# IGNF/MAESTRO

Measured on AMD Instinct MI355X. Metric: MAE-pretrain tiles/sec, higher is better.
Workload: dtype bf16

## Files before the change

maestro_amd/csrc/mask.hip:

```cpp
#include "common.hpp"
#include "../../include/maestro_hip.h"

namespace {

__global__ __launch_bounds__(1024) void mask_select_kernel(const float* __restrict__ noise, const uint8_t* __restrict__ smask,
                                                          int* __restrict__ visible_idx, int* __restrict__ masked_idx,
                                                          int* __restrict__ inv, uint8_t* __restrict__ mask, int L, int k) {
    extern __shared__ __attribute__((aligned(16))) float sm[];
    const int L4 = (L + 3) & ~3;
    int* wtot = reinterpret_cast<int*>(sm + L4);
    const int b = blockIdx.x, lane = threadIdx.x & 63, w = threadIdx.x >> 6;
    for (int i = threadIdx.x; i < L4; i += 1024) {
        float v = INFINITY;
        if (i < L) {
            v = noise[(size_t)b * L + i];
            if (smask && smask[(size_t)b * L + i]) v = 0.f;
        }
        sm[i] = v;
    }
    __syncthreads();
    int base = 0;
    for (int i0 = 0; i0 < L; i0 += 1024) {
        const int i = i0 + threadIdx.x;
        int f = 0;
// ... 32 lines not shown
                inv[(size_t)b * L + i] = i - nm;
            }
        }
    }
}

__global__ __launch_bounds__(256) void gather_rows_kernel(const float* __restrict__ src, const int* __restrict__ idx,
                                                          float* __restrict__ dst, int B, int src_L, int n_idx, int dim,
                                                          int dst_L, int dst_off) {
    const int row = blockIdx.x * 4 + (threadIdx.x >> 6), lane = threadIdx.x & 63;
    if (row >= B * n_idx) return;
    const int b = row / n_idx, j = row - b * n_idx;
    const float* s = src + ((size_t)b * src_L + idx[row]) * dim;
    float* d = dst + ((size_t)b * dst_L + dst_off + j) * dim;
    for (int c = lane * 4; c < dim; c += 256) *reinterpret_cast<f32x4*>(d + c) = *reinterpret_cast<const f32x4*>(s + c);
}

constexpr int GC_ROWS = 8;
template <int NV>
__global__ __launch_bounds__(256) void gather_rows_bf16_cs_kernel(const float* __restrict__ src, const int* __restrict__ idx,
                                                                  bf16_t* __restrict__ dst, float* __restrict__ cs_partial, int B,
                                                                  int src_L, int n_idx, int dim) {
    __shared__ f32x4 red[4][64 * NV];
    const int w = threadIdx.x >> 6, lane = threadIdx.x & 63;
    const long rows = (long)B * n_idx, row0 = ((long)blockIdx.x * 4 + w) * GC_ROWS;
    f32x4 v[GC_ROWS][NV], cs[NV];
#pragma unroll
    for (int j = 0; j < NV; ++j) cs[j] = (f32x4){0, 0, 0, 0};
#pragma unroll
    for (int r = 0; r < GC_ROWS; ++r) {
// ... 60 lines not shown
    const int row = blockIdx.x * 4 + (threadIdx.x >> 6), lane = threadIdx.x & 63;
    if (row >= B * L) return;
    const int b = row / L, t = row - b * L;
    const int iv = inv[row];
    const float* s = iv < 0 ? mask_token + (size_t)tok_slot[(size_t)b * slot_stride + t] * Dd : y + ((size_t)b * n_vis + iv) * Dd;
    const float* pr = pos + (size_t)t * Dd;
    const float* dr = date ? date + ((size_t)b * n_date_rows + date_row[t]) * 8 : nullptr;
    float* o = xdec + (size_t)row * Dd;
    for (int c = lane * 4; c < Dd; c += 256) {
        f32x4 v = *reinterpret_cast<const f32x4*>(s + c) + *reinterpret_cast<const f32x4*>(pr + c);
        if (dr && c >= Dd - 8) v += *reinterpret_cast<const f32x4*>(dr + (c - (Dd - 8)));
        *reinterpret_cast<f32x4*>(o + c) = v;
    }
}

constexpr int UM_ROWS = 512, UM_NT = 1024;
template <bool DET>
__global__ __launch_bounds__(UM_NT) void unmask_bwd_token_kernel(const float* __restrict__ dxdec, const uint8_t* __restrict__ mask,
                                                                 const int* __restrict__ tok_slot, float* __restrict__ dmask_token,
                                                                 int B, int L, int Dd, int slot, int t_lo, int t_hi, int slot_stride) {
    __shared__ __attribute__((aligned(16))) float red[UM_NT * 4];
    __shared__ int row_off[UM_ROWS];
    const int span = t_hi - t_lo, total = B * span;
    const int cols = Dd >> 2, lanes = UM_NT / cols;
    const int col = threadIdx.x % cols, sub = threadIdx.x / cols;
    const int r0 = blockIdx.x * UM_ROWS;
    for (int rr = threadIdx.x; rr < UM_ROWS; rr += UM_NT) {
        const int r = r0 + rr;
        int off = -1;
        if (r < total) {
// ... 108 lines not shown
    MH_LAUNCH_CHECK();
    return 0;
}

extern "C" int mh_unmask_assemble_per_sample(const float* y, const int* inv, const float* mask_token, const int* tok_slot_bl,
                                             const float* pos, const float* date, const int* date_row, int n_date_rows,
                                             float* xdec, int B, int L, int n_vis, int Dd, void* stream) {
    MH_CHECK_ARG(y && inv && mask_token && tok_slot_bl && pos && xdec && Dd % 4 == 0 && Dd >= 8, "mh_unmask_assemble_per_sample: bad arguments");
    MH_CHECK_ARG(!date || date_row, "mh_unmask_assemble_per_sample: date without date_row");
    hipLaunchKernelGGL(unmask_kernel, dim3(ceil_div((long)B * L, 4)), dim3(256), 0, (hipStream_t)stream, y, inv, mask_token,
                       tok_slot_bl, pos, date, date_row, n_date_rows, xdec, B, L, n_vis, Dd, L);
    MH_LAUNCH_CHECK();
    return 0;
}

extern "C" int mh_unmask_token_grad(const float* dxdec, const uint8_t* mask, const int* tok_slot, float* dmask_token, int B,
                                    int L, int Dd, int slot, int t_lo, int t_hi, void* stream) {
    MH_CHECK_ARG(dxdec && mask && tok_slot && dmask_token && Dd % 4 == 0 && Dd <= 1024, "mh_unmask_token_grad: bad arguments");
    MH_CHECK_ARG(0 <= t_lo && t_lo < t_hi && t_hi <= L, "mh_unmask_token_grad: bad token range");
    hipLaunchKernelGGL(unmask_bwd_token_kernel<false>, dim3(ceil_div((long)B * (t_hi - t_lo), UM_ROWS)), dim3(UM_NT), 0,
                       (hipStream_t)stream, dxdec, mask, tok_slot, dmask_token, B, L, Dd, slot, t_lo, t_hi, 0);
    MH_LAUNCH_CHECK();
    return 0;
}

extern "C" int mh_unmask_token_grad_per_sample(const float* dxdec, const uint8_t* mask, const int* tok_slot_bl, float* dmask_token,
                                               int B, int L, int Dd, int slot, void* stream) {
    MH_CHECK_ARG(dxdec && mask && tok_slot_bl && dmask_token && Dd % 4 == 0 && Dd <= 1024 && B > 0 && L > 0,
                 "mh_unmask_token_grad_per_sample: bad arguments");
    hipLaunchKernelGGL(unmask_bwd_token_kernel<false>, dim3(ceil_div((long)B * L, UM_ROWS)), dim3(UM_NT), 0, (hipStream_t)stream, dxdec, mask,
// ... 44 lines not shown
```

maestro_amd/csrc/norm.hip:

```cpp
#include "gemm_common.hpp"
#include <type_traits>

namespace {

struct RowMap { int L, off; };
__device__ __forceinline__ size_t map_row(RowMap m, int b, int j) { return (size_t)b * m.L + m.off + j; }

template <int NV>
__global__ __launch_bounds__(256) void ln_fwd_kernel(const float* __restrict__ x, RowMap xm, const float* __restrict__ gamma,
                                                     const float* __restrict__ beta, void* __restrict__ y, RowMap ym,
                                                     int y_is_f32, float* __restrict__ mean, float* __restrict__ rstd,
                                                     int B, int n, int dim, float eps, uint8_t* __restrict__ y8,
                                                     const float* __restrict__ y8_scale, float* __restrict__ y8_amax,
                                                     uint8_t* __restrict__ y8s, int ld_y8s) {
    const int row = blockIdx.x * 4 + (threadIdx.x >> 6);
    const int lane = threadIdx.x & 63;
    if (row >= B * n) return;
    const int b = row / n, j = row - b * n;
    const float* xr = x + map_row(xm, b, j) * dim;
    const int nv = dim >> 2;
    f32x4 v[NV];
    float s = 0.f;
#pragma unroll
    for (int i = 0; i < NV; ++i) {
// ... 121 lines not shown
            *reinterpret_cast<uint32_t*>(y8 + yrow + 4 * (lane + 64 * i)) = pack_e4m3x4(q, mx_inv_scale(sbyte));
            if ((lane & 7) == 0) y8s[map_row(ym, b, j) * ld_y8s + ((lane + 64 * i) >> 3)] = (uint8_t)sbyte;
        }
        if constexpr (FP8) {
#pragma unroll
            for (int e = 0; e < 4; ++e) amax8 = amax_fold(amax8, o[e]);
            *reinterpret_cast<uint32_t*>(y8 + yrow + 4 * (lane + 64 * i)) = pack_e4m3x4(o, s8);
        }
    }
    if (lane == 0) { mean[row] = mu; rstd[row] = rs; }
    if constexpr (FP8) {
        if (y8_amax) {
            amax8 = wave_amax(amax8);
            if (lane == 0 && amax_nonzero(amax8)) atomic_max_pos(y8_amax, amax8);
        }
    }
}

constexpr int ROWS_PER_WAVE = 4;

template <int NV, bool FULL>
__device__ __forceinline__ void ln_bwd_store_partial(float* red, float* __restrict__ partial, const f32x4 (&gsum)[NV],
                                                     const f32x4 (&bsum)[NV], const f32x4 (&csum)[NV], int w, int lane, int dim) {
    float* rg = red + (size_t)w * 3 * dim;
#pragma unroll
    for (int i = 0; i < NV; ++i) {
        const int c = lane + 64 * i;
        if (FULL || c < (dim >> 2)) {
            *reinterpret_cast<f32x4*>(rg + 4 * c) = gsum[i];
            *reinterpret_cast<f32x4*>(rg + dim + 4 * c) = bsum[i];
// ... 281 lines not shown
    MH_CHECK_ARG(!y8s || (dim % 32 == 0 && !y_is_f32), "mh_layernorm_fwd_mx: dim %% 32 == 0 required, got %d", dim);
    if (nvs <= 4 && dim == 256 * nvs && !y_is_f32) {
        auto fast = [&](auto y8_form) {
            ln_for_nv<false>(nvs, [&](auto nv) {
                hipLaunchKernelGGL((ln_fwd_fast_kernel<decltype(nv)::value, decltype(y8_form)::value>), grid, block, 0, s, x, xm, gamma,
                                   beta, (bf16_t*)y, ym, mean, rstd, B, n, eps, (uint8_t*)y8, y8_scale, y8_amax, (uint8_t*)y8s, ld_y8s);
            });
        };
        if (y8s) fast(ln_c<LN_Y8_MX>{}); else if (y8) fast(ln_c<LN_Y8_TENSOR>{}); else fast(ln_c<LN_Y8_NONE>{});
    } else {
        ln_for_nv<true>(nvs, [&](auto nv) {
            hipLaunchKernelGGL(ln_fwd_kernel<decltype(nv)::value>, grid, block, 0, s, x, xm, gamma, beta, y, ym, y_is_f32, mean, rstd, B, n,
                               dim, eps, (uint8_t*)y8, y8_scale, y8_amax, (uint8_t*)y8s, ld_y8s);
        });
    }
    MH_LAUNCH_CHECK();
    return 0;
}

extern "C" long mh_layernorm_bwd_workspace(int rows, int dim) {
    return (long)ceil_div(rows, 4 * ROWS_PER_WAVE) * 3 * dim;
}

static int layernorm_bwd_impl(const void* dy, int dy_L, int dy_off, int dy_is_f32, const float* x, int x_L, int x_off,
                              const float* gamma, const float* mean, const float* rstd, const float* dres, float* dx,
                              void* dx_bf16, float* dgamma, float* dbeta, float* dcol, float* workspace, bool partial_only,
                              int B, int n, int dim, void* stream) {
    const int rows = B * n, nblk = ceil_div(rows, 4 * ROWS_PER_WAVE);
    const size_t lds = (size_t)4 * 3 * dim * sizeof(float);
    dim3 grid(nblk), block(256);
// ... 61 lines not shown
```

maestro_amd/engine.py:

```python

from __future__ import annotations

import contextlib
import gc
import os
import weakref
import time

import torch
from torch import nn

from maestro_amd import hip
from maestro_amd.fp8 import mx_scale_cols, resolve_scaling
from maestro_amd.layers.utils import check_device_mask_config, draw_struct_masks, mask_draw_jobs

F32, BF16, I32, U8 = torch.float32, torch.bfloat16, torch.int32, torch.uint8
_NEVER = object()
_ROCTX = os.environ.get("MAESTRO_ROCTX", "0") == "1"
RING = 4
ALIGN = 64


class ParamStore:

# ... 133 lines not shown
    @property
    def x0(self):
        return self.xs[0]

    @property
    def x_last(self):
        return self.xs[-1]

    @property
    def top16(self):
        return self.saved[-1]["gy16"] if self.depth else self.dx0_16

    def top_bias_grad(self):
        return self.eng.store.g(self.t.layers[-1][1].net[4].bias) if self.depth else None

    def forward(self, before_layer=None) -> None:
        eng, ps, M = self.eng, self.eng.store, self.M
        dim, mlp, inner = self.dim, self.mlp, self.inner
        for l, (attn, ff) in enumerate(self.t.layers):
            if before_layer is not None:
                before_layer(l)
            s, x_in, x_mid, x_out = self.saved[l], self.xs[2 * l], self.xs[2 * l + 1], self.xs[2 * l + 2]
            if self.f8 is not None:
                self._forward_layer_fp8(l, attn, ff, s, x_in, x_mid, x_out)
                continue
            proj = attn.to_out[0]
            hip.layernorm_fwd(x_in, M, 0, attn.norm.weight, attn.norm.bias, s["h1"], M, 0, s["mean1"], s["rstd1"], 1, M, dim)
            hip.gemm(hip.GEMM_NT, M, 3 * inner, dim, s["h1"], dim, ps.h(attn.to_qkv.weight), dim, s["qkv"], 3 * inner)
            hip.attn_fwd(s["qkv"], s["o"], s["lse"], self.Bn, self.N, self.H, self.Dh, attn.scale)
            hip.gemm(hip.GEMM_NT, M, dim, inner, s["o"], inner, ps.h(proj.weight), inner, x_mid, dim,
                     hip.OUT_F32 | hip.BIAS | hip.RESIDUAL, bias=proj.bias, res=x_in, ldr=dim)
            ln2, fc1, fc2 = ff.net[0], ff.net[1], ff.net[4]
            hip.layernorm_fwd(x_mid, M, 0, ln2.weight, ln2.bias, s["h2"], M, 0, s["mean2"], s["rstd2"], 1, M, dim)
            hip.gemm(hip.GEMM_NT, M, mlp, dim, s["h2"], dim, ps.h(fc1.weight), dim, s["act"], mlp,
                     hip.BIAS | hip.GELU | hip.AUX_DGELU | eng.aux_flag, bias=fc1.bias, aux_out=s["hpre"], ldaux=mlp)
            hip.gemm(hip.GEMM_NT, M, dim, mlp, s["act"], mlp, ps.h(fc2.weight), mlp, x_out, dim,
                     hip.OUT_F32 | hip.BIAS | hip.RESIDUAL, bias=fc2.bias, res=x_mid, ldr=dim)

    def _forward_layer_fp8(self, l, attn, ff, s, x_in, x_mid, x_out) -> None:
        eng, M, dim, mlp, inner = self.eng, self.M, self.dim, self.mlp, self.inner
        plan, f = eng.fp8, self.f8[l]
        proj, ln2, fc1, fc2 = attn.to_out[0], ff.net[0], ff.net[1], ff.net[4]
# ... 243 lines not shown

def resolve_deterministic(flag: bool | None = None) -> bool:
    if flag is None:
        return os.environ.get("MAESTRO_DETERMINISTIC", "0") == "1"
    return bool(flag)


def resolve_mask_rng(mode: str | None = None) -> str:
    if mode is None:
        mode = os.environ.get("MAESTRO_MASK_RNG") or "host"
    if mode not in ("host", "device"):
        raise ValueError(f"mask_rng={mode!r}: expected 'host' or 'device'")
    return mode


def training_warm_passes() -> int:
    return 0 if _PROCESS_WARMED else max(0, int(os.environ.get("MAESTRO_WARM_PASSES", "6")))


def _retire_graphs(graphs: dict) -> None:
    if graphs:
        _RETIRED_GRAPHS.append(dict(graphs))
        graphs.clear()


def drain_retired_graphs() -> None:
    if _RETIRED_GRAPHS:
        torch.cuda.synchronize()
        _RETIRED_GRAPHS.clear()

# ... 355 lines not shown
        for name in m.enc_to_dec:
            ordered += [(f"enc_to_dec.{name}.{k}", p) for k, p in m.enc_to_dec[name].named_parameters()]
        ordered += [(f"mask_token.{k}", p) for k, p in m.mask_token.items()]
        for name in m.decoder:
            ordered += [(f"decoder.{name}.{k}", p) for k, p in m.decoder[name].named_parameters()]
        for name in m.embed_to_rec:
            ordered += [(f"embed_to_rec.{name}.{k}", p) for k, p in m.embed_to_rec[name].named_parameters()]
        self.store = ParamStore(ordered, device)
        for bname in ("enc_pos_encoding", "dec_pos_encoding"):
            setattr(m, bname, getattr(m, bname).to(device))
        if dtype == "fp8":
            from maestro_amd.fp8 import Fp8Plan
            self.fp8 = Fp8Plan(device, self.store.total, scaling=self.fp8_scaling)
        self._alloc()
        self._alloc_mask_upload()
        if self.fp8 is not None:
            self.fp8.finalize()
        self.store.refresh_half(force=True)
        self._pack_conv_weights()

    @property
    def grad_hook(self):
        return self._grad_hook

    @grad_hook.setter
    def grad_hook(self, fn) -> None:
        if fn is not None and getattr(self, "deterministic", False):
            raise ValueError("deterministic=True excludes a gradient hook / exchange: the order of the cross-rank sum is the "
                             "collective library's, and the ready spans would have to move behind the ordered reduce")
        self._grad_hook = fn
# ... 58 lines not shown
        for g in self.groups:
            Bn, L, N = g.Beff, g.L, g.N
            n_dates = sum(s.D for s in g.mods)
            tok_slot = torch.cat([torch.full((s.n_tok,), s.slot, dtype=I32) for s in g.mods])
            date_row = torch.cat([(s.date_off + torch.arange(s.n_tok) // s.L).to(I32) for s in g.mods])
            pos_dec = torch.cat([m.pos_dec_rows[s.name].repeat(s.D, 1) for s in g.mods], dim=0)
            self.gb[g.name] = dict(
                xg=e(Bn, L, E),
                vis=e(Bn, N, dt=I32), msk=e(Bn, g.k, dt=I32), inv=e(Bn, L, dt=I32), mask=e(Bn, L, dt=U8),
                dates=z(Bn, n_dates, 8), n_dates=n_dates, tok_slot=tok_slot.to(dev), date_row=date_row.to(dev),
                pos_dec=pos_dec.to(dev).contiguous(), tok_table=e(len(g.mods), Dd),
                henc=e(Bn * N, E, dt=BF16), mean_e=e(Bn * N), rstd_e=e(Bn * N), y_e2d=e(Bn * N, Dd),
                dy_e2d=e(Bn * N, Dd), dy_e2d16=e(Bn * N, Dd, dt=BF16), dhenc=e(Bn * N, E, dt=BF16),
                e2d_cs=e(hip.gather_rows_cs_rows(Bn * N), Dd) if self.ends_capable and Dd <= 1024 else None,
                mean_j=e(Bn * N), rstd_j=e(Bn * N))
            holder = m.encoder[g.model]
            self.enc[g.name] = Stack(self, holder, Bn, N, f"enc.{g.name}")
            self.dec[g.name] = Stack(self, m.decoder[g.model], Bn, L, f"dec.{g.name}")
        if m.encoder_inter is not None:
            self.joint = Stack(self, m.encoder_inter, self.B, m.joint_N, "joint")
        else:
            self.joint = None
        for g in self.groups:
            self.gb[g.name]["ln_ws"] = e(max(hip.layernorm_bwd_workspace(g.Beff * g.L, Dd),
                                             hip.layernorm_bwd_workspace(g.Beff * g.N, E)))
        self.loss_acc = z(1)
        srcs = {s.src: s for s in self.mods.values()}
        tot_w = sum(s.Dates * s.L for s in srcs.values())
        self.loss_w = {n: (s.Dates * s.L) / tot_w for n, s in srcs.items()}

    def _alloc_mask_upload(self) -> None:
        segs, off = [], 0
        for g in self.groups:
            for key, dt, esz in (("noise", F32, 4), ("struct", U8, 1)):
                n = g.Beff * g.L * esz
                segs.append((g.name, key, dt, off, n, (g.Beff, g.L)))
                off += (n + 255) // 256 * 256
        self._mask_dev = torch.zeros(off, dtype=U8, device=self.device)
        self._mask_segs = segs
        for name, key, dt, o, n, shape in segs:
            self.gb[name][key] = self._mask_dev[o: o + n].view(dt).view(shape)
        self._mask_stage = self._mask_host = self._upload_stream = self._mask_draw = None
        if self.mask_rng == "device":
            self._mask_draw = hip.MaskDraw(mask_draw_jobs(self.groups, self.mods, self.B),
# ... 237 lines not shown
                part = torch.empty(hip.masked_loss_partial_size(s.Beff, s.n_tok), dtype=F32, device=self.device)
                return part, [(part, self.loss_acc, part.numel(), 1, 1)]
            form, acc = "_det", self.sites.get("fwd", ("loss", s.name), make)
        elif self._loss_cs and b.get("drec_cs") is not None:
            form, cs = "_cs", (b["drec_cs"],)
        bands = () if s.G == 1 else (s.C_src, s.c0, s.C)
        getattr(hip, f"masked_loss{'_bands' if bands else ''}{form}")(
            b["rec"], b["target"], gbuf["mask"], b["cnt"], self.loss_w[s.src], acc, b["drec"], *cs, s.Beff, s.n_tok, g.L, s.tok_off,
            s.K, self.p_loss, *bands)

    def _forward_launches(self, batch: dict) -> None:
        m, E, Dd = self.model, self.E, self.Dd
        self.loss_acc.zero_()
        if self._opt is not None:
            self._opt_launch_stages()

        def head(g):
            def run():
                gbuf, st = self.gb[g.name], self.enc[g.name]
                self._opt_wait("embed")
                for s in g.mods:
                    self.embed[s.name].forward(batch, gbuf, gbuf["xg"], g.L, self.mb[s.name]["target"], self.normalise)
                hip.mask_select(gbuf["noise"], gbuf["struct"], gbuf["vis"], gbuf["msk"], gbuf["inv"], gbuf["mask"], g.Beff,
                                g.L, g.k)
                hip.gather_rows(gbuf["xg"], gbuf["vis"], st.x0, g.Beff, g.L, g.N, E, g.N, 0)
                st.forward(lambda l: self._opt_wait("enc", l))
                head_post(g, gbuf, st)
            return run

        def head_post(g, gbuf, st):
            nrm = st.t.norm
            self._opt_wait("enc", max(st.depth - 1, 0))
            if self.joint is not None:
                hip.layernorm_fwd(st.x_last, g.N, 0, nrm.weight, nrm.bias, self.joint.x0, m.joint_N, g.joint_off,
                                  gbuf["mean_e"], gbuf["rstd_e"], g.Beff, g.N, E)
            else:
                hip.layernorm_fwd(st.x_last, g.N, 0, nrm.weight, nrm.bias, gbuf["y_e2d" if self.e2d_identity else "henc"], g.N, 0,
                                  gbuf["mean_e"], gbuf["rstd_e"], g.Beff, g.N, E)

        def tail(g):
            def run():
                gbuf, st = self.gb[g.name], self.dec[g.name]
                self._opt_wait("e2d")
                if self.joint is not None:
                    nrm = self.joint.t.norm
                    hip.layernorm_fwd(self.joint.x_last, m.joint_N, g.joint_off, nrm.weight, nrm.bias,
                                      gbuf["y_e2d" if self.e2d_identity else "henc"], g.N, 0, gbuf["mean_j"], gbuf["rstd_j"],
                                      g.Beff, g.N, E)
                lin = m.enc_to_dec[g.model]
                M = g.Beff * g.N
                if not self.e2d_identity:
                    hip.gemm(hip.GEMM_NT, M, Dd, E, gbuf["henc"], E, self.store.h(lin.weight), E, gbuf["y_e2d"], Dd,
                             hip.OUT_F32 | hip.BIAS, bias=lin.bias)
                for s in g.mods:
                    gbuf["tok_table"][s.slot].copy_(m.mask_token[s.src].view(s.G, Dd)[s.gi])
                if self.tie_order == "torch":
                    hip.unmask_assemble_per_sample(gbuf["y_e2d"], gbuf["inv"], gbuf["tok_table"], gbuf["tok_slot_ps"], gbuf["pos_dec"],
                                                   gbuf["dates"], gbuf["date_row"], gbuf["n_dates"], st.x0, g.Beff, g.L, g.N, Dd)
                else:
                    hip.unmask_assemble(gbuf["y_e2d"], gbuf["inv"], gbuf["tok_table"], gbuf["tok_slot"], gbuf["pos_dec"],
                                        gbuf["dates"], gbuf["date_row"], gbuf["n_dates"], st.x0, g.Beff, g.L, g.N, Dd)
                st.forward(lambda l: self._opt_wait("dec", l))
                tail_post(g, gbuf, st)
            return run

        def tail_post(g, gbuf, st):
            nrm = st.t.norm
            self._opt_wait("rec")
            for s in g.mods:
                b = self.mb[s.name]
                T = s.Beff * s.n_tok
                conv = m.embed_to_rec[s.embed].pixelify_bands[s.gi].conv
                hip.layernorm_fwd(st.x_last, g.L, s.tok_off, nrm.weight, nrm.bias, b["hdec"], s.n_tok, 0, b["mean_f"],
                                  b["rstd_f"], s.Beff, s.n_tok, Dd)
                hip.gemm(hip.GEMM_NT, T, s.K, Dd, b["hdec"], Dd, self.store.h(conv.weight).view(s.K, Dd), Dd, b["rec"],
                         s.K, hip.OUT_F32 | hip.BIAS, bias=conv.bias)
                if s.G == 1:
                    hip.count_masked(gbuf["mask"], g.Beff, g.L, s.tok_off, s.tok_off + s.n_tok, b["cnt"])
            for s in g.mods:
                self._loss_launch(g, gbuf, s)

        self._run_parallel([head(g) for g in self.groups])
        if self.joint is not None:
            self.joint.forward(lambda l: self._opt_wait("joint", l))
        for parts in m.src_specs.values():
            if len(parts) > 1:
                for s in parts:
                    g = m.group_specs[s.group]
                    hip.count_masked_elems(self.gb[g.name]["mask"], g.Beff, g.L, s.tok_off, s.tok_off + s.n_tok,
                                           self.mb[s.name]["cnt"], s.K, s.gi > 0)
        self._run_parallel([tail(g) for g in self.groups])
        if self.deterministic:
            self._det_reduce("fwd")
        if self._opt is not None and self._opt_events:
            torch.cuda.current_stream().wait_stream(self._opt_stream)
        if self.fp8 is not None:
            self.fp8.end_of_forward()

    def zero_grad(self) -> None:
# ... 395 lines not shown
```

maestro_amd/hip.py:

```python

from __future__ import annotations

import contextlib
import ctypes
import math
import os
from pathlib import Path

import torch

_LIB_PATH = Path(__file__).resolve().parent / "lib" / "libmaestro_hip.so"
_lib = None

GEMM_NT, GEMM_NN, GEMM_TN = 0, 1, 2
OUT_F32, BIAS, GELU, RESIDUAL, DGELU, ATOMIC, COLSUM, AUX_DGELU, MULAUX, C8_E5M2, AUX_U8 = 1, 2, 4, 8, 16, 32, 64, 128, 256, 512, 1024


class HipExtensionError(RuntimeError):
    pass


def lib() -> ctypes.CDLL:
    global _lib
    if _lib is None:
# ... 345 lines not shown
def layernorm_fwd(x, x_L, x_off, gamma, beta, y, y_L, y_off, mean, rstd, B, n, dim, eps=1e-5):
    _hbm_call(f"ln_fwd<{dim}>", float(B) * n * dim * (4 + _esz(y)), "mh_layernorm_fwd", x, _I(x_L), _I(x_off), gamma, beta, y, _I(y_L),
              _I(y_off), _I(1 if y.dtype == torch.float32 else 0), mean, rstd, _I(B), _I(n), _I(dim), _F(eps))


def layernorm_fwd_fp8(x, x_L, x_off, gamma, beta, y, y_L, y_off, mean, rstd, B, n, dim, y8, y8_scale, y8_amax, eps=1e-5):
    call("mh_layernorm_fwd_fp8", x, _I(x_L), _I(x_off), gamma, beta, y, _I(y_L), _I(y_off), mean, rstd, _I(B), _I(n), _I(dim),
         _F(eps), y8, y8_scale, y8_amax)


def layernorm_fwd_mx(x, x_L, x_off, gamma, beta, y, y_L, y_off, mean, rstd, B, n, dim, y8, y8_scales, ld_y8s, eps=1e-5):
    call("mh_layernorm_fwd_mx", x, _I(x_L), _I(x_off), gamma, beta, y, _I(y_L), _I(y_off), mean, rstd, _I(B), _I(n), _I(dim),
         _F(eps), y8, y8_scales, _I(ld_y8s))


def layernorm_bwd_workspace(rows, dim) -> int:
    return int(lib().mh_layernorm_bwd_workspace(_I(rows), _I(dim)))


def layernorm_bwd(dy, dy_L, dy_off, x, x_L, x_off, gamma, mean, rstd, dres, dx, dx_bf16, dgamma, dbeta, dcol, workspace,
                  B, n, dim):
    _hbm_call(f"ln_bwd<{dim}>", float(B) * n * dim * (_esz(dy) + 4 + _esz(dres) + 4 + _esz(dx_bf16)), "mh_layernorm_bwd", dy, _I(dy_L),
              _I(dy_off), _I(1 if dy.dtype == torch.float32 else 0), x, _I(x_L), _I(x_off), gamma, mean, rstd, dres, dx, dx_bf16,
              dgamma, dbeta, dcol, workspace, _I(B), _I(n), _I(dim))


def layernorm_bwd_partial(dy, dy_L, dy_off, x, x_L, x_off, gamma, mean, rstd, dres, dx, dx_bf16, workspace, B, n, dim):
    _hbm_call(f"ln_bwd<{dim}>", float(B) * n * dim * (_esz(dy) + 4 + _esz(dres) + 4 + _esz(dx_bf16)), "mh_layernorm_bwd_partial", dy,
              _I(dy_L), _I(dy_off), _I(1 if dy.dtype == torch.float32 else 0), x, _I(x_L), _I(x_off), gamma, mean, rstd, dres, dx,
              dx_bf16, workspace, _I(B), _I(n), _I(dim))
# ... 401 lines not shown
    call("mh_expand_rows", src, inv, dst, _I(B), _I(L), _I(n), _I(dim))


def unmask_assemble(y, inv, mask_token, tok_slot, pos, date, date_row, n_date_rows, xdec, B, L, n_vis, Dd):
    call("mh_unmask_assemble", y, inv, mask_token, tok_slot, pos, date, date_row, _I(n_date_rows), xdec, _I(B), _I(L),
         _I(n_vis), _I(Dd))


def unmask_token_grad(dxdec, mask, tok_slot, dmask_token, B, L, Dd, slot, t_lo, t_hi):
    call("mh_unmask_token_grad", dxdec, mask, tok_slot, dmask_token, _I(B), _I(L), _I(Dd), _I(slot), _I(t_lo), _I(t_hi))


def unmask_assemble_per_sample(y, inv, mask_token, tok_slot_bl, pos, date, date_row, n_date_rows, xdec, B, L, n_vis, Dd):
    call("mh_unmask_assemble_per_sample", y, inv, mask_token, tok_slot_bl, pos, date, date_row, _I(n_date_rows), xdec, _I(B), _I(L),
         _I(n_vis), _I(Dd))


def unmask_token_grad_per_sample(dxdec, mask, tok_slot_bl, dmask_token, B, L, Dd, slot):
    call("mh_unmask_token_grad_per_sample", dxdec, mask, tok_slot_bl, dmask_token, _I(B), _I(L), _I(Dd), _I(slot))


def count_masked(mask, B, L, t_lo, t_hi, out):
    call("mh_count_masked", mask, _I(B), _I(L), _I(t_lo), _I(t_hi), out)


def count_masked_elems(mask, B, L, t_lo, t_hi, out, mult, accumulate):
    call("mh_count_masked_elems", mask, _I(B), _I(L), _I(t_lo), _I(t_hi), out, _I(mult), _I(int(accumulate)))


def masked_loss_bands(rec, target, mask_group, n_elems, weight, acc, drec, B, Lm, Lgroup, tok_off, PPC, p, tgt_C, tgt_c0, n_g):
# ... 1044 lines not shown
```

Measured before the change: 1906.

## Fuse first-layer LayerNorm into gather, unmask-assemble and encoder-to-joint norm kernels

Adds fused kernels that compute the first transformer block's LayerNorm (bf16 output plus mean/rstd) while rows are gathered for the encoder, while decoder inputs are assembled, and chained after the encoder's final norm into the joint stack. Stacks are then told to skip their own first ln1. The aim is to avoid re-reading activations from HBM and to drop separate launches. The decoder path also reads mask tokens through a pointer table instead of copying them into a token table on every step. It adds an environment toggle, enabled by default when fp8 is off, and it depends on the mask-token parameters keeping stable addresses.

```diff
diff --git a/maestro_amd/csrc/joins_abi.hpp b/maestro_amd/csrc/joins_abi.hpp
--- /dev/null
+++ b/maestro_amd/csrc/joins_abi.hpp
@@ -0,0 +1,26 @@
+#pragma once
+#include <stdint.h>
+
+#ifdef __cplusplus
+extern "C" {
+#endif
+
+int mh_gather_layernorm(const float* src, const int* idx, float* x0, int B, int src_L, int n_idx, int dim, const float* gamma,
+                        const float* beta, void* h16, float* mean, float* rstd, float eps, void* stream);
+
+int mh_unmask_assemble_layernorm(const float* y, const int* inv, const float* const* tok_rows, const int* tok_slot, const float* pos,
+                                 const float* date, const int* date_row, int n_date_rows, float* xdec, int B, int L, int n_vis,
+                                 int Dd, const float* gamma, const float* beta, void* h16, float* mean, float* rstd, float eps,
+                                 void* stream);
+int mh_unmask_assemble_per_sample_layernorm(const float* y, const int* inv, const float* const* tok_rows, const int* tok_slot_bl,
+                                            const float* pos, const float* date, const int* date_row, int n_date_rows,
+                                            float* xdec, int B, int L, int n_vis, int Dd, const float* gamma, const float* beta,
+                                            void* h16, float* mean, float* rstd, float eps, void* stream);
+
+int mh_layernorm_fwd_chain(const float* x, int x_L, int x_off, const float* gamma, const float* beta, float* y, int y_L, int y_off,
+                           float* mean, float* rstd, float eps, const float* gamma2, const float* beta2, void* h2, float* mean2,
+                           float* rstd2, float eps2, int B, int n, int dim, void* stream);
+
+#ifdef __cplusplus
+}
+#endif
diff --git a/maestro_amd/csrc/ln_row.hpp b/maestro_amd/csrc/ln_row.hpp
--- /dev/null
+++ b/maestro_amd/csrc/ln_row.hpp
@@ -0,0 +1,99 @@
+#pragma once
+#include "common.hpp"
+
+#define MH_LN_ROW_EXACT _Pragma("clang fp contract(off)")
+
+static inline int ln_row_nv(int dim) { const int v = (dim / 4 + 63) / 64; return v <= 4 ? v : 8; }
+static inline bool ln_row_fast(int dim) { const int v = ln_row_nv(dim); return v <= 4 && dim == 256 * v; }
+template <class F>
+static void ln_row_dispatch(int dim, F&& f) {
+    const bool fast = ln_row_fast(dim);
+    switch (ln_row_nv(dim)) {
+#define MH_LN_ROW_CASE(V) case V: if (fast) f(std::integral_constant<int, V>{}, std::true_type{}); \
+                                  else f(std::integral_constant<int, V>{}, std::false_type{}); break
+        MH_LN_ROW_CASE(1); MH_LN_ROW_CASE(2); MH_LN_ROW_CASE(3); MH_LN_ROW_CASE(4);
+#undef MH_LN_ROW_CASE
+        default: f(std::integral_constant<int, 8>{}, std::false_type{});
+    }
+}
+
+__device__ __forceinline__ float ln_row_wave_sum(float v) {
+#define MH_ROR(n) __builtin_bit_cast(float, __builtin_amdgcn_update_dpp(0, __builtin_bit_cast(int, v), 0x120 + (n), 0xf, 0xf, false))
+    v += MH_ROR(8); v += MH_ROR(4); v += MH_ROR(2); v += MH_ROR(1);
+#undef MH_ROR
+    const int iv = __builtin_bit_cast(int, v);
+    const float r0 = __builtin_bit_cast(float, __builtin_amdgcn_readlane(iv, 0)), r1 = __builtin_bit_cast(float, __builtin_amdgcn_readlane(iv, 16));
+    const float r2 = __builtin_bit_cast(float, __builtin_amdgcn_readlane(iv, 32)), r3 = __builtin_bit_cast(float, __builtin_amdgcn_readlane(iv, 48));
+    return (r0 + r1) + (r2 + r3);
+}
+
+template <int NV>
+__device__ __forceinline__ void ln_row_pin(f32x4 (&v)[NV]) {
+#pragma unroll
+    for (int i = 0; i < NV; ++i) {
+#pragma unroll
+        for (int e = 0; e < 4; ++e) { float t = v[i][e]; asm volatile("" : "+v"(t)); v[i][e] = t; }
+    }
+}
+
+template <int NV>
+__device__ __forceinline__ void ln_row_fwd_fast(const f32x4 (&v)[NV], const f32x4 (&g)[NV], const f32x4 (&bt)[NV], bf16_t* __restrict__ yr,
+                                                float* __restrict__ mean_p, float* __restrict__ rstd_p, int lane, float eps) {
+    MH_LN_ROW_EXACT
+    constexpr int dim = 256 * NV;
+    float s = 0.f;
+#pragma unroll
+    for (int i = 0; i < NV; ++i) s += (v[i][0] + v[i][1]) + (v[i][2] + v[i][3]);
+    const float mu = ln_row_wave_sum(s) / dim;
+    float q = 0.f;
+#pragma unroll
+    for (int i = 0; i < NV; ++i) {
+#pragma unroll
+        for (int e = 0; e < 4; ++e) { const float d = v[i][e] - mu; q += d * d; }
+    }
+    const float rs = rsqrtf(ln_row_wave_sum(q) / dim + eps);
+#pragma unroll
+    for (int i = 0; i < NV; ++i) {
+        f32x4 o;
+#pragma unroll
+        for (int e = 0; e < 4; ++e) o[e] = __builtin_fmaf((v[i][e] - mu) * rs, g[i][e], bt[i][e]);
+        const u32x2 pk = {pack_bf2(o[0], o[1]), pack_bf2(o[2], o[3])};
+        *reinterpret_cast<u32x2*>(yr + 4 * (lane + 64 * i)) = pk;
+    }
+    if (lane == 0) { *mean_p = mu; *rstd_p = rs; }
+}
+
+template <int NV>
+__device__ __forceinline__ void ln_row_fwd_generic(const f32x4 (&v)[NV], const float* __restrict__ gamma, const float* __restrict__ beta,
+                                                   bf16_t* __restrict__ yr, float* __restrict__ mean_p, float* __restrict__ rstd_p,
+                                                   int lane, int dim, float eps) {
+    MH_LN_ROW_EXACT
+    const int nv = dim >> 2;
+    float s = 0.f;
+#pragma unroll
+    for (int i = 0; i < NV; ++i) s += (v[i][0] + v[i][1]) + (v[i][2] + v[i][3]);
+    const float mu = wave_sum(s) / dim;
+    float q = 0.f;
+#pragma unroll
+    for (int i = 0; i < NV; ++i) {
+        if (lane + 64 * i < nv) {
+#pragma unroll
+            for (int e = 0; e < 4; ++e) { const float d = v[i][e] - mu; q += d * d; }
+        }
+    }
+    const float rs = rsqrtf(wave_sum(q) / dim + eps);
+    if (lane == 0) { *mean_p = mu; *rstd_p = rs; }
+#pragma unroll
+    for (int i = 0; i < NV; ++i) {
+        const int c = lane + 64 * i;
+        if (c < nv) {
+            const f32x4 g = *reinterpret_cast<const f32x4*>(gamma + 4 * c);
+            const f32x4 bt = *reinterpret_cast<const f32x4*>(beta + 4 * c);
+            f32x4 o;
+#pragma unroll
+            for (int e = 0; e < 4; ++e) o[e] = __builtin_fmaf((v[i][e] - mu) * rs, g[e], bt[e]);
+            const u32x2 pk = {pack_bf2(o[0], o[1]), pack_bf2(o[2], o[3])};
+            *reinterpret_cast<u32x2*>(yr + 4 * c) = pk;
+        }
+    }
+}
diff --git a/maestro_amd/csrc/mask.hip b/maestro_amd/csrc/mask.hip
--- a/maestro_amd/csrc/mask.hip
+++ b/maestro_amd/csrc/mask.hip
@@ -1,4 +1,6 @@
 #include "common.hpp"
+#include "joins_abi.hpp"
+#include "ln_row.hpp"
 #include "../../include/maestro_hip.h"
 
 namespace {
@@ -70,6 +72,46 @@
     const float* s = src + ((size_t)b * src_L + idx[row]) * dim;
     float* d = dst + ((size_t)b * dst_L + dst_off + j) * dim;
     for (int c = lane * 4; c < dim; c += 256) *reinterpret_cast<f32x4*>(d + c) = *reinterpret_cast<const f32x4*>(s + c);
+}
+
+template <int NV, bool FAST>
+__global__ __launch_bounds__(256) void gather_ln_kernel(const float* __restrict__ src, const int* __restrict__ idx,
+                                                        float* __restrict__ dst, const float* __restrict__ gamma,
+                                                        const float* __restrict__ beta, bf16_t* __restrict__ h16,
+                                                        float* __restrict__ mean, float* __restrict__ rstd, int B, int src_L,
+                                                        int n_idx, int dim, float eps) {
+    const int row = blockIdx.x * 4 + __builtin_amdgcn_readfirstlane(threadIdx.x >> 6), lane = threadIdx.x & 63;
+    if (row >= B * n_idx) return;
+    const int b = row / n_idx;
+    const float* s = src + ((size_t)b * src_L + idx[row]) * dim;
+    float* d = dst + (size_t)row * dim;
+    bf16_t* yr = h16 + (size_t)row * dim;
+    f32x4 v[NV];
+    if constexpr (FAST) {
+        f32x4 g[NV], bt[NV];
+#pragma unroll
+        for (int i = 0; i < NV; ++i) v[i] = *reinterpret_cast<const f32x4*>(s + 4 * (lane + 64 * i));
+#pragma unroll
+        for (int i = 0; i < NV; ++i) {
+            g[i] = *reinterpret_cast<const f32x4*>(gamma + 4 * (lane + 64 * i));
+            bt[i] = *reinterpret_cast<const f32x4*>(beta + 4 * (lane + 64 * i));
+        }
+#pragma unroll
+        for (int i = 0; i < NV; ++i) *reinterpret_cast<f32x4*>(d + 4 * (lane + 64 * i)) = v[i];
+        ln_row_fwd_fast<NV>(v, g, bt, yr, mean + row, rstd + row, lane, eps);
+    } else {
+        const int nv = dim >> 2;
+#pragma unroll
+        for (int i = 0; i < NV; ++i) {
+            const int c = lane + 64 * i;
+            v[i] = (f32x4){0, 0, 0, 0};
+            if (c < nv) {
+                v[i] = *reinterpret_cast<const f32x4*>(s + 4 * c);
+                *reinterpret_cast<f32x4*>(d + 4 * c) = v[i];
+            }
+        }
+        ln_row_fwd_generic<NV>(v, gamma, beta, yr, mean + row, rstd + row, lane, dim, eps);
+    }
 }
 
 constexpr int GC_ROWS = 8;
@@ -160,6 +202,47 @@
     }
 }
 
+template <int NV, bool FAST>
+__global__ __launch_bounds__(256) void unmask_ln_kernel(const float* __restrict__ y, const int* __restrict__ inv,
+                                                        const float* const* __restrict__ tok_rows, const int* __restrict__ tok_slot,
+                                                        const float* __restrict__ pos, const float* __restrict__ date,
+                                                        const int* __restrict__ date_row, int n_date_rows, float* __restrict__ xdec,
+                                                        const float* __restrict__ gamma, const float* __restrict__ beta,
+                                                        bf16_t* __restrict__ h16, float* __restrict__ mean, float* __restrict__ rstd,
+                                                        int B, int L, int n_vis, int Dd, int slot_stride, float eps) {
+    const int row = blockIdx.x * 4 + __builtin_amdgcn_readfirstlane(threadIdx.x >> 6), lane = threadIdx.x & 63;
+    if (row >= B * L) return;
+    const int b = row / L, t = row - b * L;
+    const int iv = inv[row];
+    const float* s = iv < 0 ? tok_rows[tok_slot[(size_t)b * slot_stride + t]] : y + ((size_t)b * n_vis + iv) * Dd;
+    const float* pr = pos + (size_t)t * Dd;
+    const float* dr = date ? date + ((size_t)b * n_date_rows + date_row[t]) * 8 : nullptr;
+    float* o = xdec + (size_t)row * Dd;
+    bf16_t* yr = h16 + (size_t)row * Dd;
+    f32x4 v[NV];
+    [[maybe_unused]] f32x4 g[NV], bt[NV];
+    if constexpr (FAST) {
+#pragma unroll
+        for (int i = 0; i < NV; ++i) {
+            g[i] = *reinterpret_cast<const f32x4*>(gamma + 4 * (lane + 64 * i));
+            bt[i] = *reinterpret_cast<const f32x4*>(beta + 4 * (lane + 64 * i));
+        }
+    }
+#pragma unroll
+    for (int i = 0; i < NV; ++i) {
+        const int c = 4 * (lane + 64 * i);
+        v[i] = (f32x4){0, 0, 0, 0};
+        if (FAST || c < Dd) {
+            v[i] = *reinterpret_cast<const f32x4*>(s + c) + *reinterpret_cast<const f32x4*>(pr + c);
+            if (dr && c >= Dd - 8) v[i] += *reinterpret_cast<const f32x4*>(dr + (c - (Dd - 8)));
+            *reinterpret_cast<f32x4*>(o + c) = v[i];
+        }
+    }
+    ln_row_pin(v);
+    if constexpr (FAST) ln_row_fwd_fast<NV>(v, g, bt, yr, mean + row, rstd + row, lane, eps);
+    else ln_row_fwd_generic<NV>(v, gamma, beta, yr, mean + row, rstd + row, lane, Dd, eps);
+}
+
 constexpr int UM_ROWS = 512, UM_NT = 1024;
 template <bool DET>
 __global__ __launch_bounds__(UM_NT) void unmask_bwd_token_kernel(const float* __restrict__ dxdec, const uint8_t* __restrict__ mask,
@@ -298,6 +381,55 @@
     return 0;
 }
 
+extern "C" int mh_gather_layernorm(const float* src, const int* idx, float* x0, int B, int src_L, int n_idx, int dim, const float* gamma,
+                                   const float* beta, void* h16, float* mean, float* rstd, float eps, void* stream) {
+    MH_CHECK_ARG(src && idx && x0 && gamma && beta && h16 && mean && rstd, "mh_gather_layernorm: null pointer");
+    MH_CHECK_ARG(B > 0 && src_L > 0 && n_idx > 0 && n_idx <= src_L && dim % 4 == 0 && dim >= 8 && dim <= 2048,
+                 "mh_gather_layernorm: bad sizes B=%d src_L=%d n_idx=%d dim=%d (dim %% 4 == 0, 8 <= dim <= 2048)", B, src_L, n_idx, dim);
+    const dim3 grid(ceil_div((long)B * n_idx, 4)), block(256);
+    ln_row_dispatch(dim, [&](auto nv, auto fast) {
+        hipLaunchKernelGGL((gather_ln_kernel<decltype(nv)::value, decltype(fast)::value>), grid, block, 0, (hipStream_t)stream, src, idx,
+                           x0, gamma, beta, (bf16_t*)h16, mean, rstd, B, src_L, n_idx, dim, eps);
+    });
+    MH_LAUNCH_CHECK();
+    return 0;
+}
+
+static int unmask_layernorm(const char* name, const float* y, const int* inv, const float* const* tok_rows, const int* tok_slot,
+                            int slot_stride, const float* pos, const float* date, const int* date_row, int n_date_rows, float* xdec,
+                            int B, int L, int n_vis, int Dd, const float* gamma, const float* beta, void* h16, float* mean, float* rstd,
+                            float eps, void* stream) {
+    MH_CHECK_ARG(y && inv && tok_rows && tok_slot && pos && xdec && gamma && beta && h16 && mean && rstd, "%s: null pointer", name);
+    MH_CHECK_ARG(!date || date_row, "%s: date without date_row", name);
+    MH_CHECK_ARG(B > 0 && L > 0 && n_vis > 0 && Dd % 4 == 0 && Dd >= 8 && Dd <= 2048,
+                 "%s: bad sizes B=%d L=%d n_vis=%d Dd=%d (Dd %% 4 == 0, 8 <= Dd <= 2048)", name, B, L, n_vis, Dd);
+    const dim3 grid(ceil_div((long)B * L, 4)), block(256);
+    ln_row_dispatch(Dd, [&](auto nv, auto fast) {
+        hipLaunchKernelGGL((unmask_ln_kernel<decltype(nv)::value, decltype(fast)::value>), grid, block, 0, (hipStream_t)stream, y, inv,
+                           tok_rows, tok_slot, pos, date, date_row, n_date_rows, xdec, gamma, beta, (bf16_t*)h16, mean, rstd, B, L,
+                           n_vis, Dd, slot_stride, eps);
+    });
+    MH_LAUNCH_CHECK();
+    return 0;
+}
+
+extern "C" int mh_unmask_assemble_layernorm(const float* y, const int* inv, const float* const* tok_rows, const int* tok_slot,
+                                            const float* pos, const float* date, const int* date_row, int n_date_rows, float* xdec,
+                                            int B, int L, int n_vis, int Dd, const float* gamma, const float* beta, void* h16,
+                                            float* mean, float* rstd, float eps, void* stream) {
+    return unmask_layernorm("mh_unmask_assemble_layernorm", y, inv, tok_rows, tok_slot, 0, pos, date, date_row, n_date_rows, xdec, B, L,
+                            n_vis, Dd, gamma, beta, h16, mean, rstd, eps, stream);
+}
+
+extern "C" int mh_unmask_assemble_per_sample_layernorm(const float* y, const int* inv, const float* const* tok_rows,
+                                                       const int* tok_slot_bl, const float* pos, const float* date,
+                                                       const int* date_row, int n_date_rows, float* xdec, int B, int L, int n_vis,
+                                                       int Dd, const float* gamma, const float* beta, void* h16, float* mean,
+                                                       float* rstd, float eps, void* stream) {
+    return unmask_layernorm("mh_unmask_assemble_per_sample_layernorm", y, inv, tok_rows, tok_slot_bl, L, pos, date, date_row,
+                            n_date_rows, xdec, B, L, n_vis, Dd, gamma, beta, h16, mean, rstd, eps, stream);
+}
+
 extern "C" int mh_unmask_token_grad(const float* dxdec, const uint8_t* mask, const int* tok_slot, float* dmask_token, int B,
                                     int L, int Dd, int slot, int t_lo, int t_hi, void* stream) {
     MH_CHECK_ARG(dxdec && mask && tok_slot && dmask_token && Dd % 4 == 0 && Dd <= 1024, "mh_unmask_token_grad: bad arguments");
diff --git a/maestro_amd/csrc/norm.hip b/maestro_amd/csrc/norm.hip
--- a/maestro_amd/csrc/norm.hip
+++ b/maestro_amd/csrc/norm.hip
@@ -1,4 +1,6 @@
 #include "gemm_common.hpp"
+#include "joins_abi.hpp"
+#include "ln_row.hpp"
 #include <type_traits>
 
 namespace {
@@ -159,6 +161,67 @@
             amax8 = wave_amax(amax8);
             if (lane == 0 && amax_nonzero(amax8)) atomic_max_pos(y8_amax, amax8);
         }
+    }
+}
+
+template <int NV, bool FAST2>
+__global__ __launch_bounds__(256) void ln_fwd_chain_kernel(const float* __restrict__ x, RowMap xm, const float* __restrict__ gamma,
+                                                           const float* __restrict__ beta, float* __restrict__ y, RowMap ym,
+                                                           float* __restrict__ mean, float* __restrict__ rstd, float eps,
+                                                           const float* __restrict__ gamma2, const float* __restrict__ beta2,
+                                                           bf16_t* __restrict__ h2, float* __restrict__ mean2,
+                                                           float* __restrict__ rstd2, float eps2, int B, int n, int dim) {
+    MH_LN_ROW_EXACT
+    const int row = blockIdx.x * 4 + (threadIdx.x >> 6);
+    const int lane = threadIdx.x & 63;
+    if (row >= B * n) return;
+    const int b = row / n, j = row - b * n;
+    const float* xr = x + map_row(xm, b, j) * dim;
+    const int nv = dim >> 2;
+    f32x4 v[NV], o[NV];
+    float s = 0.f;
+#pragma unroll
+    for (int i = 0; i < NV; ++i) {
+        const int c = lane + 64 * i;
+        v[i] = (f32x4){0, 0, 0, 0};
+        if (c < nv) v[i] = *reinterpret_cast<const f32x4*>(xr + 4 * c);
+        s += (v[i][0] + v[i][1]) + (v[i][2] + v[i][3]);
+    }
+    const float mu = wave_sum(s) / dim;
+    float q = 0.f;
+#pragma unroll
+    for (int i = 0; i < NV; ++i) {
+        if (lane + 64 * i < nv) {
+#pragma unroll
+            for (int e = 0; e < 4; ++e) { const float d = v[i][e] - mu; q += d * d; }
+        }
+    }
+    const float rs = rsqrtf(wave_sum(q) / dim + eps);
+    if (lane == 0) { mean[row] = mu; rstd[row] = rs; }
+    const size_t r2 = map_row(ym, b, j);
+#pragma unroll
+    for (int i = 0; i < NV; ++i) {
+        const int c = lane + 64 * i;
+        o[i] = (f32x4){0, 0, 0, 0};
+        if (c < nv) {
+            const f32x4 g = *reinterpret_cast<const f32x4*>(gamma + 4 * c);
+            const f32x4 bt = *reinterpret_cast<const f32x4*>(beta + 4 * c);
+#pragma unroll
+            for (int e = 0; e < 4; ++e) o[i][e] = __builtin_fmaf((v[i][e] - mu) * rs, g[e], bt[e]);
+            *reinterpret_cast<f32x4*>(y + r2 * dim + 4 * c) = o[i];
+        }
+    }
+    ln_row_pin(o);
+    if constexpr (FAST2) {
+        f32x4 g2[NV], bt2[NV];
+#pragma unroll
+        for (int i = 0; i < NV; ++i) {
+            g2[i] = *reinterpret_cast<const f32x4*>(gamma2 + 4 * (lane + 64 * i));
+            bt2[i] = *reinterpret_cast<const f32x4*>(beta2 + 4 * (lane + 64 * i));
+        }
+        ln_row_fwd_fast<NV>(o, g2, bt2, h2 + r2 * dim, mean2 + r2, rstd2 + r2, lane, eps2);
+    } else {
+        ln_row_fwd_generic<NV>(o, gamma2, beta2, h2 + r2 * dim, mean2 + r2, rstd2 + r2, lane, dim, eps2);
     }
 }
 
@@ -470,6 +533,23 @@
                                dim, eps, (uint8_t*)y8, y8_scale, y8_amax, (uint8_t*)y8s, ld_y8s);
         });
     }
+    MH_LAUNCH_CHECK();
+    return 0;
+}
+
+extern "C" int mh_layernorm_fwd_chain(const float* x, int x_L, int x_off, const float* gamma, const float* beta, float* y, int y_L,
+                                      int y_off, float* mean, float* rstd, float eps, const float* gamma2, const float* beta2, void* h2,
+                                      float* mean2, float* rstd2, float eps2, int B, int n, int dim, void* stream) {
+    MH_CHECK_ARG(x && gamma && beta && y && mean && rstd && gamma2 && beta2 && h2 && mean2 && rstd2, "mh_layernorm_fwd_chain: null pointer");
+    MH_CHECK_ARG(dim % 4 == 0 && dim >= 4 && dim <= 2048, "mh_layernorm_fwd_chain: dim %d unsupported", dim);
+    MH_CHECK_ARG(B > 0 && n > 0 && x_off >= 0 && y_off >= 0 && x_off + n <= x_L && y_off + n <= y_L, "mh_layernorm_fwd_chain: bad row map");
+    MH_CHECK_ARG((const void*)x != (const void*)y, "mh_layernorm_fwd_chain: out of place only");
+    const dim3 grid(ceil_div((long)B * n, 4)), block(256);
+    const RowMap xm{x_L, x_off}, ym{y_L, y_off};
+    ln_row_dispatch(dim, [&](auto nv, auto fast2) {
+        hipLaunchKernelGGL((ln_fwd_chain_kernel<decltype(nv)::value, decltype(fast2)::value>), grid, block, 0, (hipStream_t)stream, x, xm,
+                           gamma, beta, y, ym, mean, rstd, eps, gamma2, beta2, (bf16_t*)h2, mean2, rstd2, eps2, B, n, dim);
+    });
     MH_LAUNCH_CHECK();
     return 0;
 }
diff --git a/maestro_amd/engine.py b/maestro_amd/engine.py
--- a/maestro_amd/engine.py
+++ b/maestro_amd/engine.py
@@ -171,9 +171,14 @@
     def top_bias_grad(self):
         return self.eng.store.g(self.t.layers[-1][1].net[4].bias) if self.depth else None
 
-    def forward(self, before_layer=None) -> None:
+    def ln1_of_first_layer(self) -> tuple:
+        norm, s = self.t.layers[0][0].norm, self.saved[0]
+        return norm.weight, norm.bias, s["h1"], s["mean1"], s["rstd1"]
+
+    def forward(self, before_layer=None, ln1_done: bool = False) -> None:
         eng, ps, M = self.eng, self.eng.store, self.M
         dim, mlp, inner = self.dim, self.mlp, self.inner
+        assert not (ln1_done and self.f8 is not None), "the fp8 forward's LayerNorm also writes e4m3 copies: no join"
         for l, (attn, ff) in enumerate(self.t.layers):
             if before_layer is not None:
                 before_layer(l)
@@ -182,7 +187,8 @@
                 self._forward_layer_fp8(l, attn, ff, s, x_in, x_mid, x_out)
                 continue
             proj = attn.to_out[0]
-            hip.layernorm_fwd(x_in, M, 0, attn.norm.weight, attn.norm.bias, s["h1"], M, 0, s["mean1"], s["rstd1"], 1, M, dim)
+            if not (ln1_done and l == 0):
+                hip.layernorm_fwd(x_in, M, 0, attn.norm.weight, attn.norm.bias, s["h1"], M, 0, s["mean1"], s["rstd1"], 1, M, dim)
             hip.gemm(hip.GEMM_NT, M, 3 * inner, dim, s["h1"], dim, ps.h(attn.to_qkv.weight), dim, s["qkv"], 3 * inner)
             hip.attn_fwd(s["qkv"], s["o"], s["lse"], self.Bn, self.N, self.H, self.Dh, attn.scale)
             hip.gemm(hip.GEMM_NT, M, dim, inner, s["o"], inner, ps.h(proj.weight), inner, x_mid, dim,
@@ -456,6 +462,19 @@
     return mode
 
 
+JOIN_EMBED, JOIN_JOINT, JOIN_DECODER = 1, 2, 4
+
+
+def resolve_fwd_joins(value: str | None = None) -> int:
+    value = os.environ.get("MAESTRO_FWD_JOINS", "1") if value is None else value
+    every = JOIN_EMBED | JOIN_JOINT | JOIN_DECODER
+    if value in ("0", "1"):
+        return every if value == "1" else 0
+    if value.lower().startswith("0x") and 0 <= int(value, 16) <= every:
+        return int(value, 16)
+    raise ValueError(f"MAESTRO_FWD_JOINS={value!r}: expected 0, 1 or a bit set 0x0 .. {every:#x}")
+
+
 def training_warm_passes() -> int:
     return 0 if _PROCESS_WARMED else max(0, int(os.environ.get("MAESTRO_WARM_PASSES", "6")))
 
@@ -841,6 +860,7 @@
             self.fp8 = Fp8Plan(device, self.store.total, scaling=self.fp8_scaling)
         self._alloc()
         self._alloc_mask_upload()
+        self.fwd_joins = resolve_fwd_joins() if self.fp8 is None else 0
         if self.fp8 is not None:
             self.fp8.finalize()
         self.store.refresh_half(force=True)
@@ -929,6 +949,8 @@
                 dy_e2d=e(Bn * N, Dd), dy_e2d16=e(Bn * N, Dd, dt=BF16), dhenc=e(Bn * N, E, dt=BF16),
                 e2d_cs=e(hip.gather_rows_cs_rows(Bn * N), Dd) if self.ends_capable and Dd <= 1024 else None,
                 mean_j=e(Bn * N), rstd_j=e(Bn * N))
+            rows = self._mask_token_rows(g)
+            self.gb[g.name].update(tok_rows=hip.token_row_table(rows, dev), tok_rows_host=[r.data_ptr() for r in rows])
             holder = m.encoder[g.model]
             self.enc[g.name] = Stack(self, holder, Bn, N, f"enc.{g.name}")
             self.dec[g.name] = Stack(self, m.decoder[g.model], Bn, L, f"dec.{g.name}")
@@ -943,6 +965,14 @@
         srcs = {s.src: s for s in self.mods.values()}
         tot_w = sum(s.Dates * s.L for s in srcs.values())
         self.loss_w = {n: (s.Dates * s.L) / tot_w for n, s in srcs.items()}
+
+    def _mask_token_rows(self, g) -> list:
+        return [self.model.mask_token[s.src].data.view(s.G, self.Dd)[s.gi] for s in g.mods]
+
+    def _tok_rows(self, g, gbuf) -> torch.Tensor:
+        if gbuf["tok_rows_host"] != [r.data_ptr() for r in self._mask_token_rows(g)]:
+            raise hip.HipExtensionError(f"group {g.name}: a mask token no longer lives in the engine's flat parameter store")
+        return gbuf["tok_rows"]
 
     def _alloc_mask_upload(self) -> None:
         segs, off = [], 0
@@ -1210,6 +1240,8 @@
         self.loss_acc.zero_()
         if self._opt is not None:
             self._opt_launch_stages()
+        joins = self.fwd_joins
+        join_joint = bool(joins & JOIN_JOINT) and self.joint is not None and self.joint.depth > 0
 
         def head(g):
             def run():
@@ -1219,15 +1251,24 @@
                     self.embed[s.name].forward(batch, gbuf, gbuf["xg"], g.L, self.mb[s.name]["target"], self.normalise)
                 hip.mask_select(gbuf["noise"], gbuf["struct"], gbuf["vis"], gbuf["msk"], gbuf["inv"], gbuf["mask"], g.Beff,
                                 g.L, g.k)
-                hip.gather_rows(gbuf["xg"], gbuf["vis"], st.x0, g.Beff, g.L, g.N, E, g.N, 0)
-                st.forward(lambda l: self._opt_wait("enc", l))
+                if joins & JOIN_EMBED and st.depth:
+                    self._opt_wait("enc", 0)
+                    hip.gather_layernorm(gbuf["xg"], gbuf["vis"], st.x0, g.Beff, g.L, g.N, E, *st.ln1_of_first_layer())
+                    st.forward(lambda l: self._opt_wait("enc", l), ln1_done=True)
+                else:
+                    hip.gather_rows(gbuf["xg"], gbuf["vis"], st.x0, g.Beff, g.L, g.N, E, g.N, 0)
+                    st.forward(lambda l: self._opt_wait("enc", l))
                 head_post(g, gbuf, st)
             return run
 
         def head_post(g, gbuf, st):
             nrm = st.t.norm
             self._opt_wait("enc", max(st.depth - 1, 0))
-            if self.joint is not None:
+            if self.joint is not None and join_joint:
+                self._opt_wait("joint", 0)
+                hip.layernorm_fwd_chain(st.x_last, g.N, 0, nrm.weight, nrm.bias, self.joint.x0, m.joint_N, g.joint_off,
+                                        gbuf["mean_e"], gbuf["rstd_e"], *self.joint.ln1_of_first_layer(), g.Beff, g.N, E)
+            elif self.joint is not None:
                 hip.layernorm_fwd(st.x_last, g.N, 0, nrm.weight, nrm.bias, self.joint.x0, m.joint_N, g.joint_off,
                                   gbuf["mean_e"], gbuf["rstd_e"], g.Beff, g.N, E)
             else:
@@ -1248,9 +1289,19 @@
                 if not self.e2d_identity:
                     hip.gemm(hip.GEMM_NT, M, Dd, E, gbuf["henc"], E, self.store.h(lin.weight), E, gbuf["y_e2d"], Dd,
                              hip.OUT_F32 | hip.BIAS, bias=lin.bias)
+                per_sample = self.tie_order == "torch"
+                if joins & JOIN_DECODER and st.depth:
+                    self._opt_wait("dec", 0)
+                    hip.unmask_assemble_layernorm(gbuf["y_e2d"], gbuf["inv"], self._tok_rows(g, gbuf),
+                                                  gbuf["tok_slot_ps" if per_sample else "tok_slot"], gbuf["pos_dec"], gbuf["dates"],
+                                                  gbuf["date_row"], gbuf["n_dates"], st.x0, g.Beff, g.L, g.N, Dd,
+                                                  *st.ln1_of_first_layer(), per_sample=per_sample)
+                    st.forward(lambda l: self._opt_wait("dec", l), ln1_done=True)
+                    tail_post(g, gbuf, st)
+                    return
                 for s in g.mods:
                     gbuf["tok_table"][s.slot].copy_(m.mask_token[s.src].view(s.G, Dd)[s.gi])
-                if self.tie_order == "torch":
+                if per_sample:
                     hip.unmask_assemble_per_sample(gbuf["y_e2d"], gbuf["inv"], gbuf["tok_table"], gbuf["tok_slot_ps"], gbuf["pos_dec"],
                                                    gbuf["dates"], gbuf["date_row"], gbuf["n_dates"], st.x0, g.Beff, g.L, g.N, Dd)
                 else:
@@ -1278,7 +1329,7 @@
 
         self._run_parallel([head(g) for g in self.groups])
         if self.joint is not None:
-            self.joint.forward(lambda l: self._opt_wait("joint", l))
+            self.joint.forward(lambda l: self._opt_wait("joint", l), ln1_done=join_joint)
         for parts in m.src_specs.values():
             if len(parts) > 1:
                 for s in parts:
diff --git a/maestro_amd/hip.py b/maestro_amd/hip.py
--- a/maestro_amd/hip.py
+++ b/maestro_amd/hip.py
@@ -383,6 +383,12 @@
          _F(eps), y8, y8_scales, _I(ld_y8s))
 
 
+def layernorm_fwd_chain(x, x_L, x_off, gamma, beta, y, y_L, y_off, mean, rstd, gamma2, beta2, h2, mean2, rstd2, B, n, dim,
+                        eps=1e-5, eps2=1e-5):
+    call("mh_layernorm_fwd_chain", x, _I(x_L), _I(x_off), gamma, beta, y, _I(y_L), _I(y_off), mean, rstd, _F(eps), gamma2, beta2, h2,
+         mean2, rstd2, _F(eps2), _I(B), _I(n), _I(dim))
+
+
 def layernorm_bwd_workspace(rows, dim) -> int:
     return int(lib().mh_layernorm_bwd_workspace(_I(rows), _I(dim)))
 
@@ -814,6 +820,23 @@
 def unmask_assemble_per_sample(y, inv, mask_token, tok_slot_bl, pos, date, date_row, n_date_rows, xdec, B, L, n_vis, Dd):
     call("mh_unmask_assemble_per_sample", y, inv, mask_token, tok_slot_bl, pos, date, date_row, _I(n_date_rows), xdec, _I(B), _I(L),
          _I(n_vis), _I(Dd))
+
+
+def gather_layernorm(src, idx, x0, B, src_L, n_idx, dim, gamma, beta, h16, mean, rstd, eps=1e-5):
+    call("mh_gather_layernorm", src, idx, x0, _I(B), _I(src_L), _I(n_idx), _I(dim), gamma, beta, h16, mean, rstd, _F(eps))
+
+
+def token_row_table(rows, device) -> torch.Tensor:
+    for r in rows:
+        if not (r.is_cuda and r.dtype == torch.float32 and r.is_contiguous()):
+            raise HipExtensionError("token_row_table: contiguous fp32 GPU rows expected")
+    return torch.tensor([r.data_ptr() for r in rows], dtype=torch.int64).to(device)
+
+
+def unmask_assemble_layernorm(y, inv, tok_rows, tok_slot, pos, date, date_row, n_date_rows, xdec, B, L, n_vis, Dd, gamma, beta,
+                              h16, mean, rstd, per_sample=False, eps=1e-5):
+    call("mh_unmask_assemble_per_sample_layernorm" if per_sample else "mh_unmask_assemble_layernorm", y, inv, tok_rows, tok_slot,
+         pos, date, date_row, _I(n_date_rows), xdec, _I(B), _I(L), _I(n_vis), _I(Dd), gamma, beta, h16, mean, rstd, _F(eps))
 
 
 def unmask_token_grad_per_sample(dxdec, mask, tok_slot_bl, dmask_token, B, L, Dd, slot):
```

Result: no change. 1911 (median of 2 runs) (+0.3%).
